# Atten4Vis/LW-DETR

Hardware: AMD Instinct MI355X
Metric: images/sec (higher is better)
Workload: dtype fp16; 1 GPU; LW-DETR-small inference forward + PostProcess, 640x640, batch 32/GPU, fp16, random-init weights (synthetic COCO-shaped input); global_batch=32, per_gpu_batch=32, parallelism=dp1, collective=none, launch_chains=2

## Files before the change

include/lwdetr_hip.h:

```cpp
#ifndef LWDETR_HIP_H
#define LWDETR_HIP_H
#include <stdint.h>
#ifdef __cplusplus
extern "C" {
#endif

#define LWDETR_OK 0
#define LWDETR_ERR_BAD_ARG (-1)
#define LWDETR_ERR_UNSUPPORTED (-2)
#define LWDETR_ERR_LAUNCH (-3)

int lwdetr_msda_forward(const void* value, const int64_t* shapes, const int64_t* level_start, const void* loc,
                        const void* attn, void* out, int B, int S, int M, int D, int L, int Q, int P, int dtype,
                        void* hip_stream);

int lwdetr_msda_backward(const void* value, const int64_t* shapes, const int64_t* level_start, const void* loc,
                         const void* attn, const void* grad_out, void* grad_value, void* grad_loc, void* grad_attn,
                         int B, int S, int M, int D, int L, int Q, int P, int dtype, void* hip_stream);

int lwdetr_msda_fused_forward(const void* value, const int64_t* shapes, const int64_t* level_start, const void* oa,
                              long ld_oa, int logit_col, const float* ref_boxes, const float* valid_ratios, void* out,
                              int B, int S, int M, int D, int L, int Q, int P, int dtype, void* hip_stream);

typedef struct {
    int winmajor;
    int Hp, Wp, Twp;
} lwdetr_tok_layout;

enum { LWDETR_A_PLAIN = 0, LWDETR_A_CONV3x3 = 1, LWDETR_A_PATCH16 = 2 };
enum { LWDETR_ACT_NONE = 0, LWDETR_ACT_RELU = 1, LWDETR_ACT_GELU = 2, LWDETR_ACT_SILU = 3 };
enum { LWDETR_OUT_LINEAR = 0, LWDETR_OUT_HEADS = 1, LWDETR_OUT_HEADS_T = 2, LWDETR_OUT_TOKMAP = 3,
       LWDETR_OUT_DECONV2x2 = 4 };

typedef struct {
    void* out;
    void* out2;
    const void* res;
    const float* bias;
    const float* gamma;
    const uint8_t* rowmask;
    float scale;
    int act;
    int mode;
    int n_begin, n_end;
    long ldo, ld2, ldres;
    int res_mod;
    int rowmask_after;
    int p0, p1, p2;
    lwdetr_tok_layout in_tok, out_tok;
    long out_batch_stride;
    long out_row_offset;
    const float* ln_stats;
    const float* ln_colsum;
} lwdetr_gemm_seg;

typedef struct {
    const void* A; const void* A2;
    const void* W;
    int M, N, K;
    long lda;
    int a_mode;
    lwdetr_tok_layout a_tok;
    int conv_cin, conv_stride, a_col0, conv_hout, conv_wout;
    int img_h, img_w;
    int nseg;
    lwdetr_gemm_seg seg[3];
    void* splitk_ws;
    int splitk;
} lwdetr_gemm_desc;

int lwdetr_gemm(const lwdetr_gemm_desc* desc, int dtype, void* hip_stream);
int lwdetr_gemm_few(const lwdetr_gemm_desc* desc, int dtype, void* hip_stream);
int lwdetr_row_stats(const void* x, long ldx, long M, int C, float eps, float* stats, int dtype, void* hip_stream);
void lwdetr_gemm_tuning(int big_mode);
int lwdetr_has_experiments(void);
void lwdetr_gemm_pt_tuning(int pt_mode);
long lwdetr_gemm_pt_count(void);
int lwdetr_gemm_path_counts(long* out, int n);
const char* lwdetr_gemm_path_name(int i);

typedef struct {
    const void* Q;
    const void* K;
    const void* VT;
    void* out;
    long ldo;
    int B, heads, hd, Tp;
    int seqs_per_img;
    int seq_tok_stride;
    int keys_per_seq;
    int sub_stride, sub_len;
    int kind;
    int vt_slack;
} lwdetr_attn_desc;

int lwdetr_attention(const lwdetr_attn_desc* desc, int dtype, void* hip_stream);
void lwdetr_attention_tuning(int lds_mode);
void lwdetr_attention_tuning_cfg(int cfg);

int lwdetr_layernorm(const void* x, long ldx, const float* gamma, const float* beta, void* out, long ldo, long M,
                     int C, float eps, long rows_per_batch, long out_batch_rows, long out_row_offset, int dtype,
                     void* hip_stream);

int lwdetr_layernorm_chain(const void* x, long ldx, const float* gamma1, const float* beta1, float eps1, void* out1, long ldo1,
                           const float* gamma2, const float* beta2, float eps2, void* out2, long ldo2, long M, int C,
                           int dtype, void* hip_stream);

int lwdetr_ffn_splits(long M, int C, int hid, int dtype);
int lwdetr_ffn_partial(const void* x, long ldx, const void* w1, const float* b1, const void* w2_chunked, float* partial, long M,
                       int C, int hid, int dtype, void* hip_stream);
int lwdetr_ffn_finish(const void* x, long ldx, const float* partial, int splits, const float* b2, const float* gamma1,
                      const float* beta1, float eps1, void* out1, long ldo1, const float* gamma2, const float* beta2, float eps2,
                      void* out2, long ldo2, long M, int C, int dtype, void* hip_stream);

int lwdetr_mlp_fused(void* x, long ldx, const void* w1_folded, const float* b1_folded, const void* w2_chunked,
                     const float* b2, const float* gamma2, void* out2, long ld2, float* stats_out, long M, int C,
                     float eps, float eps_next, const void* att, long ldatt, const void* wp, const float* bp,
                     const float* gamma1, const void* wqkv_next, const float* bqkv_next, void* q_out, void* k_out,
                     void* vt_out, float qscale, int heads, int hd, int Tp, int dtype, void* hip_stream);

int lwdetr_vit_block_few(void* x, long ldx, const void* w1_frag, const float* b1_folded, const void* w2_chunked, const float* b2,
                         const float* gamma2, void* out2, long ld2, float* stats_out, long M, int C, float eps, float eps_next,
                         const void* att, long ldatt, const void* wp_frag, const float* bp, const float* gamma1,
                         const void* wqkv_frag_next, const float* bqkv_next, void* q_out, void* k_out, void* vt_out, float qscale,
                         int heads, int hd, int Tp, int dtype, void* hip_stream);

int lwdetr_vit_path_counts(long* out, int n);
const char* lwdetr_vit_path_name(int i);

int lwdetr_msda_path_counts(long* out, int n);
const char* lwdetr_msda_path_name(int i);
long lwdetr_vit_block_stream_bytes(int C, int has_qkv);
long lwdetr_vit_block_vec_floats(int C);
int lwdetr_vit_block(void* x, long ldx, const void* att, long ldatt, const void* wstream, const float* vec, void* out2,
                     long ld2, float* stats_out, long M, int C, float eps, float eps_next, int has_qkv, void* q_out,
                     void* k_out, void* vt_out, float qscale, int heads, int hd, int Tp, int dtype, void* hip_stream);

long lwdetr_enc_chain_vec_floats(int D, int k5);
long lwdetr_enc_chain_pieces(int D, int k5, int nl);
long lwdetr_enc_chain_class_cols(int ncls);
long lwdetr_enc_chain_vec_floats_cls(int D, int k5, int ncls);
long lwdetr_enc_chain_pieces_cls(int D, int k5, int nl, int ncls);
int lwdetr_enc_chain_check(const void* in, long ld_in, int k5, void* memory, void* om, void* cls, long ld_cls, float* cls_max,
                           void* const* values, int nl, const unsigned char* rowvalid, const unsigned char* notpad,
                           const void* wstream, const float* vec, long M, int D, int npix, int S, int lsi, long total_rows,
                           int ncls, int dtype);
int lwdetr_enc_chain(const void* in, long ld_in, int k5, void* memory, void* om, void* cls, long ld_cls, float* cls_max,
                     void* const* values, int nl, const unsigned char* rowvalid, const unsigned char* notpad,
                     const void* wstream, const float* vec, long M, int D, int npix, int S, int lsi, long total_rows,
                     int ncls, float eps_p, float eps_e, int dtype, void* hip_stream);

enum { LWDETR_CHAIN_FULL = 0, LWDETR_CHAIN_SIDE = 1 };
enum { LWDETR_CHAIN_RES = 1, LWDETR_CHAIN_RELU = 2, LWDETR_CHAIN_LN = 4, LWDETR_CHAIN_STORE = 8, LWDETR_CHAIN_ADDQ = 16 };
typedef struct { int kind; int n; int flags; float eps; void* out; long ldo; } lwdetr_chain_stage;
typedef struct {
    const void* in; long ld_in; int k_in;
    const void* res; long ld_res;
    const void* qpos; long ld_q;
    const void* wstream; const float* vec;
    long M; int D; int nst;
    lwdetr_chain_stage st[6];
} lwdetr_chain_desc;
long lwdetr_row_chain_pieces(const lwdetr_chain_desc* desc);
long lwdetr_row_chain_vec_floats(const lwdetr_chain_desc* desc);
int lwdetr_row_chain(const lwdetr_chain_desc* desc, int dtype, void* hip_stream);

long lwdetr_vit_qkv_stream_bytes(int C);
long lwdetr_vit_qkv_vec_floats(int C);
int lwdetr_vit_qkv(const void* x, long ldx, const void* wstream, const float* vec, long M, int C, float eps, void* q_out,
                   void* k_out, void* vt_out, float qscale, int heads, int hd, int Tp, int dtype, void* hip_stream);

long lwdetr_vit_stem_stream_bytes(int C);
long lwdetr_vit_stem_vec_floats(int C);
int lwdetr_vit_stem(const void* img, int B, int img_h, int img_w, int Hp, int Wp, int Twp, const void* pos, long ldpos, void* x,
                    long ldx, const void* wstream, const float* vec, long M, int C, float eps, void* q_out, void* k_out,
                    void* vt_out, float qscale, int heads, int hd, int dtype, void* hip_stream);

int lwdetr_select_gather(const void* om, const void* enc_cls, long ldc, const float* props, const int64_t* idx,
                         void* om_sel, void* logits_out, float* props_sel, int B, int S, int d, int nq, int ncls,
                         int dtype, void* hip_stream);
int lwdetr_decoder_inputs(const void* enc_delta, const float* props_sel, const float* refpoint, const float* valid_ratios,
                          int L, const void* query_feat, const float* dim_t, void* enc_boxes_out, float* ref_out,
                          void* sine_out, void* xdec_out, int B, int nq, int d, int dtype, void* hip_stream);
int lwdetr_box_reparam(const void* delta, const float* ref, long ref_rows, void* out, long R, int dtype, void* hip_stream);
int lwdetr_finalize_outputs(const void* delta, const float* ref, long ref_rows, void* coord_out, long R, const void* logits_pad,
                            long ldc, int ncls, void* logits_out, long out_layer_rows, int dtype, void* hip_stream);

int lwdetr_rowmax(const void* x, long ld, long rows, int ncols, float* out, int dtype, void* hip_stream);
int lwdetr_topk(const void* x, int B, int N, int K, int64_t* idx_out, float* val_out, int dtype, void* hip_stream);
int lwdetr_postprocess(const void* logits, const void* boxes, const float* target_sizes, int B, int nq, int ncls, int K,
                       float* scores, int64_t* labels, float* out_boxes, int dtype, void* hip_stream);
int lwdetr_postprocess_packed(const void* logits, const void* boxes, const float* target_sizes, int B, int nq, int ncls, int K,
                              float* packed, int dtype, void* hip_stream);

typedef struct {
    const uint8_t* src;
    int height, width;
    long row_stride;
    int xbounds_off, xcoef_off, xksize;
    int ybounds_off, ycoef_off, yksize;
    long tmp_off;
} lwdetr_resize_image;
int lwdetr_resize_normalize(const lwdetr_resize_image* images, int B, int max_height, const int32_t* tables, uint8_t* tmp,
                            const float* lut, void* out, int S, int dtype, void* hip_stream);

int lwdetr_tuning_set(const char* name, long value, int is_set);

int lwdetr_prof_enable(int on);
int lwdetr_prof_num_kernels(void);
const char* lwdetr_prof_kernel_name(int kid);
int lwdetr_prof_collect(double* ms, double* flops, double* bytes, long long* count, int n);

#ifdef __cplusplus
}
#endif
#endif
```

lw-detr_amd/csrc/attention.hip:

```cpp
#include "common.h"
#include <cstdlib>

namespace {

__device__ __forceinline__ float xor16_max(float v) {
    const auto r = __builtin_amdgcn_permlane16_swap(__float_as_uint(v), __float_as_uint(v), false, false);
    return fmaxf(__uint_as_float(r[0]), __uint_as_float(r[1]));
}
__device__ __forceinline__ float xor32_max(float v) {
    const auto r = __builtin_amdgcn_permlane32_swap(__float_as_uint(v), __float_as_uint(v), false, false);
    return fmaxf(__uint_as_float(r[0]), __uint_as_float(r[1]));
}
__device__ __forceinline__ float xor16_sum(float v) {
    const auto r = __builtin_amdgcn_permlane16_swap(__float_as_uint(v), __float_as_uint(v), false, false);
    return __uint_as_float(r[0]) + __uint_as_float(r[1]);
}
__device__ __forceinline__ float xor32_sum(float v) {
    const auto r = __builtin_amdgcn_permlane32_swap(__float_as_uint(v), __float_as_uint(v), false, false);
    return __uint_as_float(r[0]) + __uint_as_float(r[1]);
}

__device__ __forceinline__ float max3(float a, float b, float c) { return __builtin_fmaxf(__builtin_fmaxf(a, b), c); }

#ifndef LWDETR_ATTN_ABL
#define LWDETR_ATTN_ABL 0
#endif

template <typename T, int HD, int QT, bool SHORT = false>
__global__ __launch_bounds__(256) void attn_kernel(const lwdetr_attn_desc p) {
    typedef typename Vec<T>::v8 V8;
    typedef typename Vec<T>::v4 V4;
    constexpr int NC = HD >= 32 ? HD / 32 : 1;
    constexpr int DT = HD / 16;
    const int lane = threadIdx.x & 63, wave = threadIdx.x >> 6;
    const int l15 = lane & 15, g = lane >> 4;
    const int head = blockIdx.y, seq = blockIdx.z;
    const int q0 = (blockIdx.x * 4 + wave) * 16 * QT;
    if (q0 >= p.keys_per_seq) return;
    const int b = seq / p.seqs_per_img, w = seq - b * p.seqs_per_img;
    const long tok0 = (long)w * p.seq_tok_stride;
    const long bh = (long)b * p.heads + head;
    const T* __restrict__ Qb = (const T*)p.Q + (bh * p.Tp + tok0) * HD;
    const T* __restrict__ Kb = (const T*)p.K + (bh * p.Tp + tok0) * HD;
    const T* __restrict__ Vb = (const T*)p.VT + bh * HD * (long)p.Tp + tok0;
    const int nkeys = p.keys_per_seq;
    const int last = nkeys - 1;

    V8 q8[QT][NC]; V4 q4[QT];
#pragma unroll
    for (int t = 0; t < QT; ++t) {
        int q = q0 + t * 16 + l15; q = q < last ? q : last;
        if (HD >= 32) {
#pragma unroll
            for (int c = 0; c < NC; ++c) q8[t][c] = *(const V8*)(Qb + (long)q * HD + c * 32 + g * 8);
        } else {
            q4[t] = *(const V4*)(Qb + (long)q * HD + g * 4);
        }
    }

    f32x4 o[QT][DT], lsum[QT];
    f32x4 negm[QT];
#pragma unroll
    for (int t = 0; t < QT; ++t) {
        negm[t] = f32x4{0.f, 0.f, 0.f, 0.f}; lsum[t] = f32x4{0.f, 0.f, 0.f, 0.f};
#pragma unroll
        for (int dt = 0; dt < DT; ++dt) o[t][dt] = f32x4{0.f, 0.f, 0.f, 0.f};
    }
    V8 ones;
#pragma unroll
    for (int e = 0; e < 8; ++e) ones[e] = from_f32<T>(1.f);

    const bool holes = p.sub_len < p.sub_stride;
    constexpr float RESCALE_THR = 8.f;

    struct KV { V8 k8[2][NC]; V4 k4[2]; V8 v[DT]; };
    auto load_k = [&](int k0, KV& f) {
#pragma unroll
        for (int kt = 0; kt < 2; ++kt) {
            int key = k0 + 8 * (l15 >> 2) + 4 * kt + (l15 & 3); key = key < last ? key : last;
            if (HD >= 32) {
#pragma unroll
                for (int c = 0; c < NC; ++c) f.k8[kt][c] = *(const V8*)(Kb + (long)key * HD + c * 32 + g * 8);
            } else {
                f.k4[kt] = *(const V4*)(Kb + (long)key * HD + g * 4);
            }
        }
    };
    auto load_v = [&](int k0, KV& f) {
        int kv = k0 + g * 8;
        kv = kv + 7 < nkeys ? kv : (nkeys - 8);
        const bool shift4 = k0 + g * 8 - kv == 4;
#pragma unroll
        for (int dt = 0; dt < DT; ++dt) {
            V8 v = *(const V8*)(Vb + (long)(dt * 16 + l15) * p.Tp + kv);
            if (shift4) {
#pragma unroll
                for (int e = 0; e < 4; ++e) v[e] = v[4 + e];
            }
            f.v[dt] = v;
        }
    };
    auto load_kv = [&](int k0, KV& f) { load_k(k0, f); load_v(k0, f); };

    auto qk_tile = [&](const KV& f, int t, f32x4 (&st)[2]) {
#pragma unroll
        for (int kt = 0; kt < 2; ++kt) {
            f32x4 a = negm[t];
            if (LWDETR_ATTN_ABL & 4) { a[0] += to_f32<T>(f.k4[kt][0]); st[kt] = a; continue; }
            if (HD >= 32) {
#pragma unroll
                for (int c = 0; c < NC; ++c) a = Mma<T>::k32(f.k8[kt][c], q8[t][c], a);
            } else {
                a = Mma<T>::k16(f.k4[kt], q4[t], a);
            }
            st[kt] = a;
        }
    };
    auto softmax_head = [&](f32x4 (&s)[QT][2], int k0) {
        if (k0 + 32 > nkeys || holes) {
#pragma unroll
            for (int kt = 0; kt < 2; ++kt)
#pragma unroll
                for (int r = 0; r < 4; ++r) {
                    const int key = k0 + g * 8 + kt * 4 + r;
                    const int sub = holes ? key % p.sub_stride : 0;
                    const bool ok = (key < nkeys) & (sub < p.sub_len);
#pragma unroll
                    for (int t = 0; t < QT; ++t) s[t][kt][r] = ok ? s[t][kt][r] : -INFINITY;
                }
        }
        float lmax[QT];
#pragma unroll
        for (int t = 0; t < QT; ++t) {
            lmax[t] = max3(s[t][0][0], s[t][0][1], s[t][0][2]);
            lmax[t] = max3(lmax[t], s[t][0][3], s[t][1][0]);
            lmax[t] = max3(lmax[t], s[t][1][1], s[t][1][2]);
            lmax[t] = max3(lmax[t], s[t][1][3], s[t][1][3]);
        }
        if (LWDETR_ATTN_ABL & 2) { for (int t = 0; t < QT; ++t) lmax[t] = s[t][0][0]; }
        float lall = lmax[0];
#pragma unroll
        for (int t = 1; t + 1 < QT; t += 2) lall = max3(lall, lmax[t], lmax[t + 1]);
        if (QT % 2 == 0) lall = max3(lall, lmax[QT - 1], lmax[QT - 1]);
        const bool need = k0 == 0 || lall > RESCALE_THR;
        if (__any(need)) {
#pragma unroll
            for (int t = 0; t < QT; ++t) {
                float mx = xor32_max(xor16_max(lmax[t]));
                mx = k0 == 0 ? mx : fmaxf(mx, 0.f);
                const float alpha = __builtin_amdgcn_exp2f(-mx);
                negm[t] -= mx;
#pragma unroll
                for (int kt = 0; kt < 2; ++kt) s[t][kt] -= mx;
                lsum[t] *= alpha;
#pragma unroll
                for (int dt = 0; dt < DT; ++dt) o[t][dt] *= alpha;
            }
        }
    };
    auto pv_tile = [&](const KV& f, int t, const f32x4 (&st)[2]) {
        V8 pf;
#pragma unroll
        for (int kt = 0; kt < 2; ++kt)
#pragma unroll
            for (int r = 0; r < 4; ++r) {
                const float e = (LWDETR_ATTN_ABL & 1) ? st[kt][r] : __builtin_amdgcn_exp2f(st[kt][r]);
                pf[kt * 4 + r] = from_f32<T>(e);
            }
        if (LWDETR_ATTN_ABL & 8) { lsum[t][0] += to_f32<T>(pf[0]) + to_f32<T>(pf[5]); return; }
        lsum[t] = Mma<T>::k32(ones, pf, lsum[t]);
#pragma unroll
        for (int dt = 0; dt < DT; ++dt) o[t][dt] = Mma<T>::k32(f.v[dt], pf, o[t][dt]);
    };
    auto step = [&](const KV& f, int k0) {
        f32x4 s[QT][2];
#pragma unroll
        for (int t = 0; t < QT; ++t) qk_tile(f, t, s[t]);
        softmax_head(s, k0);
#pragma unroll
        for (int t = 0; t < QT; ++t) pv_tile(f, t, s[t]);
    };

    if constexpr (SHORT) {
        KV f4[4];
#pragma unroll
        for (int i = 0; i < 4; ++i) load_kv(32 * i, f4[i]);
#pragma unroll
        for (int i = 0; i < 4; ++i) {
            if (32 * i >= nkeys) break;
            step(f4[i], 32 * i);
        }
    } else {
    KV fa, fb;
    if (nkeys >= 512) {
        load_kv(0, fa);
        for (int k0 = 0;;) {
            load_kv(k0 + 32, fb);
            step(fa, k0);
            k0 += 32;
            if (k0 >= nkeys) break;
            load_kv(k0 + 32, fa);
            step(fb, k0);
            k0 += 32;
            if (k0 >= nkeys) break;
        }
    } else {
        load_kv(0, fa);
        for (int k0 = 0;;) {
            if (k0 + 32 < nkeys) load_kv(k0 + 32, fb);
            step(fa, k0);
            k0 += 32;
            if (k0 >= nkeys) break;
            if (k0 + 32 < nkeys) load_kv(k0 + 32, fa);
            step(fb, k0);
            k0 += 32;
            if (k0 >= nkeys) break;
        }
    }
    }

    T* __restrict__ out = (T*)p.out;
#pragma unroll
    for (int t = 0; t < QT; ++t) {
        const float l = lsum[t][0];
        const float inv = 1.f / l;
        const int q = q0 + t * 16 + l15;
        if (q < nkeys) {
            T* orow = out + ((long)b * p.Tp + tok0 + q) * p.ldo + head * HD;
#pragma unroll
            for (int dt = 0; dt < DT; ++dt) {
                V4 ov;
#pragma unroll
                for (int r = 0; r < 4; ++r) ov[r] = from_f32<T>(o[t][dt][r] * inv);
                *(V4*)(orow + dt * 16 + g * 4) = ov;
            }
        }
    }
}


template <typename T> struct Mma32;
template <> struct Mma32<f16> {
    static __device__ __forceinline__ f32x16 k16(f16x8 a, f16x8 b, f32x16 c) {
        return __builtin_amdgcn_mfma_f32_32x32x16_f16(a, b, c, 0, 0, 0);
    }
    static __device__ __forceinline__ float dot2(f16x8 p, int i, float c) {
        typedef _Float16 h2 __attribute__((ext_vector_type(2)));
        const h2 a = {p[2 * i], p[2 * i + 1]}, one = {(f16)1.f, (f16)1.f};
        return __builtin_amdgcn_fdot2(a, one, c, false);
    }
};
template <> struct Mma32<bf16> {
    static __device__ __forceinline__ f32x16 k16(bf16x8 a, bf16x8 b, f32x16 c) {
        return __builtin_amdgcn_mfma_f32_32x32x16_bf16(a, b, c, 0, 0, 0);
    }
    static __device__ __forceinline__ float dot2(bf16x8 p, int i, float c) {
        typedef __bf16 b2 __attribute__((ext_vector_type(2)));
        const b2 a = {p[2 * i], p[2 * i + 1]}, one = {(bf16)1.f, (bf16)1.f};
        return __builtin_amdgcn_fdot2_f32_bf16(a, one, c, false);
    }
};

__device__ __attribute__((aligned(16))) unsigned int g_attn_zero16[4];

__device__ __forceinline__ void attn_dma16(const void* src, unsigned lds_base) {
    asm volatile("s_mov_b32 m0, %0\n\ts_nop 0\n\tglobal_load_lds_dwordx4 %1, off" :: "s"(lds_base), "v"(src) : "memory");
}
template <int N> __device__ __forceinline__ void attn_wait_vmcnt() { asm volatile("s_waitcnt vmcnt(%0)" ::"n"(N) : "memory"); }

template <typename T, int HD, int QT, int NW, int U>
__global__ __launch_bounds__(NW * 64) void attn_lds_kernel(const lwdetr_attn_desc p) {
    typedef typename Vec<T>::v8 V8;
    constexpr int NC = HD / 16;
    constexpr int RT = HD > 32 ? HD / 32 : 1;
    constexpr int RB = HD * 2;
    constexpr int CPR = RB / 16, RPB = 256 / RB;
    constexpr int KB = 64;
    constexpr int KIMG = KB * RB, VIMG = RT * 32 * 128, STAGE = KIMG + VIMG;
    constexpr int NKP = KIMG / 1024, NVP = HD * 128 / 1024, NP = NKP + NVP;
    constexpr int SSTAGE = U * STAGE;
    constexpr int PPW = (U * NP + NW - 1) / NW;
    constexpr int NST = 3;
    constexpr int QW = 32 * QT, QWG = QW * NW;
    constexpr float RESCALE_THR = 8.f;
    __shared__ __attribute__((aligned(16))) char smem[NST * SSTAGE + 1024];

    const int lane = threadIdx.x & 63;
    const int wave = __builtin_amdgcn_readfirstlane(threadIdx.x >> 6);
    const int m = lane & 31, h = lane >> 5;
    const int nkeys = p.keys_per_seq;
    const int wgs_per_seq = (nkeys + QWG - 1) / QWG;
    int wid;
    {
        const int nwg = gridDim.x, bid = blockIdx.x, q = nwg >> 3, r = nwg & 7, xcd = bid & 7;
        wid = (xcd < r ? xcd * (q + 1) : r * (q + 1) + (xcd - r) * q) + (bid >> 3);
    }
    const int qblk = wid % wgs_per_seq;
    const int rest = wid / wgs_per_seq;
    const int head = rest % p.heads, seq = rest / p.heads;
    const int b = seq / p.seqs_per_img, w = seq - b * p.seqs_per_img;
    const long tok0 = (long)w * p.seq_tok_stride;
    const long bh = (long)b * p.heads + head;
    const T* __restrict__ Qb = (const T*)p.Q + (bh * p.Tp + tok0) * HD;
    const T* __restrict__ Kb = (const T*)p.K + (bh * p.Tp + tok0) * HD;
    const T* __restrict__ Vb = (const T*)p.VT + bh * HD * (long)p.Tp + tok0;
    const int q0 = qblk * QWG + wave * QW;
    const bool active = q0 < nkeys;
    const int nblk = (nkeys + KB - 1) / KB;
    const int nstep = (nblk + U - 1) / U;

    V8 qf[QT][NC];
#pragma unroll
    for (int t = 0; t < QT; ++t) {
        int q = q0 + t * 32 + m; q = q < nkeys ? q : nkeys - 1;
#pragma unroll
        for (int c = 0; c < NC; ++c) qf[t][c] = *(const V8*)(Qb + (long)q * HD + c * 16 + h * 8);
    }

    const T* src0[PPW]; const T* srct[PPW]; int sstep[PPW]; unsigned dst0[PPW]; bool real[PPW]; int sub[PPW];
    const unsigned lds0 = (unsigned)(uintptr_t)(__attribute__((address_space(3))) const void*)smem;
    const unsigned dummy_dst = lds0 + NST * SSTAGE;
    const int kt0 = (nblk - 1) * KB;
#pragma unroll
    for (int j = 0; j < PPW; ++j) {
        const int ii = wave + j * NW;
        const int i = ii % NP;
        sub[j] = ii / NP;
        if (ii >= U * NP) {
            src0[j] = (const T*)g_attn_zero16; srct[j] = src0[j]; sstep[j] = 0; dst0[j] = 0; real[j] = false;
        } else if (i < NKP) {
            const int off = i * 1024 + lane * 16;
            const int key = off / RB, slot = (off % RB) / 16;
            const int chunk = slot ^ ((key / RPB) & (CPR - 1));
            src0[j] = Kb + key * HD + chunk * 8; sstep[j] = KB * HD; dst0[j] = sub[j] * STAGE + i * 1024; real[j] = true;
            const int kc = kt0 + key < nkeys ? kt0 + key : nkeys - 1;
            srct[j] = Kb + (long)kc * HD + chunk * 8;
        } else {
            const int v = i - NKP;
            const int row = 8 * v + (lane >> 3), slot = lane & 7;
            const int chunk = slot ^ ((row >> 1) & 7);
            src0[j] = Vb + (long)row * p.Tp + chunk * 8; sstep[j] = KB; dst0[j] = sub[j] * STAGE + KIMG + v * 1024; real[j] = true;
            srct[j] = kt0 + chunk * 8 < nkeys ? src0[j] + kt0 : (const T*)g_attn_zero16;
        }
    }
    auto issue = [&](int step, int slot_) {
        const unsigned sb = lds0 + slot_ * SSTAGE;
#pragma unroll
        for (int j = 0; j < PPW; ++j) {
            const int blk = step * U + sub[j];
            const bool live = real[j] && blk < nblk;
            const T* src = !live ? (const T*)g_attn_zero16 : (blk == nblk - 1 ? srct[j] : src0[j] + (long)blk * sstep[j]);
            attn_dma16(src, __builtin_amdgcn_readfirstlane(live ? sb + dst0[j] : dummy_dst));
        }
    };

    if (HD == 16) {
        V8 one8, zero8;
#pragma unroll
        for (int e = 0; e < 8; ++e) { one8[e] = from_f32<T>(1.f); zero8[e] = from_f32<T>(0.f); }
        for (int i = threadIdx.x; i < NST * U * 16 * 8; i += NW * 64) {
            const int st = i / 128, r = (i % 128) / 8, sl = i % 8;
            *(V8*)(smem + st * STAGE + KIMG + (16 + r) * 128 + sl * 16) = r == 0 ? one8 : zero8;
        }
    }

    const int km = (m & ~12) | ((m & 4) << 1) | ((m & 8) >> 1);
    int kofs[NC];
#pragma unroll
    for (int c = 0; c < NC; ++c) kofs[c] = km * RB + (((2 * c + h) ^ ((km / RPB) & (CPR - 1))) << 4);
    int vofs[2][2];
#pragma unroll
    for (int t = 0; t < 2; ++t)
#pragma unroll
        for (int s = 0; s < 2; ++s) vofs[t][s] = KIMG + m * 128 + (((4 * t + 2 * s + h) ^ ((m >> 1) & 7)) << 4);

    f32x16 o[QT][RT], negm[QT];
    float lsum[QT];
#pragma unroll
    for (int t = 0; t < QT; ++t) {
        lsum[t] = 0.f;
#pragma unroll
        for (int e = 0; e < 16; ++e) negm[t][e] = 0.f;
#pragma unroll
        for (int r = 0; r < RT; ++r)
#pragma unroll
            for (int e = 0; e < 16; ++e) o[t][r][e] = 0.f;
    }
    const bool holes = p.sub_len < p.sub_stride;
    int res0 = 0;

// ... 384 lines not shown
    const int kid = p.kind == 0 ? KID_ATTN_WINDOW : (p.kind == 1 ? KID_ATTN_GLOBAL : KID_ATTN_DECODER);
    ProfScope ps(kid, flops, bytes, st);
    hipLaunchKernelGGL((attn_win_kernel<T, HD>), dim3((unsigned)((npairs + 3) / 4)), dim3(256), 0, st, p);
    return lwdetr_check_launch();
}

#ifdef LWDETR_EXPERIMENTS
template <typename T>
__global__ __launch_bounds__(256) void attn_wtile_kernel(const lwdetr_attn_desc p) {
    constexpr int HD = 16;
    typedef typename Vec<T>::v8 V8;
    typedef typename Vec<T>::v4 V4;
    typedef unsigned u32x4v __attribute__((ext_vector_type(4)));
    typedef unsigned u32x2 __attribute__((ext_vector_type(2)));
    static_assert(sizeof(T) == 2, "16-bit types");
    extern __shared__ __attribute__((aligned(16))) char wt_smem[];
    const int tid = threadIdx.x, lane = tid & 63, wave = tid >> 6, l31 = lane & 31, h = lane >> 5;
    const int w = (int)(blockIdx.x % (unsigned)p.seqs_per_img), b = (int)(blockIdx.x / (unsigned)p.seqs_per_img);
    const long tok0 = (long)w * p.seq_tok_stride;
    const int nkeys = p.keys_per_seq, last = nkeys - 1;
    const int nvalid = p.sub_len < nkeys ? p.sub_len : nkeys;
    const int nqt = (nkeys + 31) >> 5, nkt = (nvalid + 31) >> 5, nch = (nvalid + 15) >> 4;
    const int C = p.heads * HD;
    const int VLD = ((nkeys + 7) & ~7) + 8;
    const int OLD = C + 8;
    T* vs = (T*)wt_smem;
    T* os = vs + (size_t)C * VLD;

    auto load_qk = [&](int head, V8 (&kf)[4], V8 (&qf)[4]) {
        const long bh = (long)b * p.heads + head;
        const T* __restrict__ Qb = (const T*)p.Q + (bh * p.Tp + tok0) * HD;
        const T* __restrict__ Kb = (const T*)p.K + (bh * p.Tp + tok0) * HD;
#pragma unroll
        for (int t = 0; t < 4; ++t) {
            int r = t * 32 + l31; r = r < last ? r : last;
            kf[t] = *(const V8*)(Kb + (long)r * HD + h * 8);
            qf[t] = *(const V8*)(Qb + (long)r * HD + h * 8);
        }
    };
    V8 kf[4], qf[4];
    int head = wave;
    if (head < p.heads) load_qk(head, kf, qf);
    {
        const int ppr = nkeys >> 2, total = C * ppr;
        const T* __restrict__ Vw = (const T*)p.VT + (long)b * C * (long)p.Tp + tok0;
        for (int i = tid; i < total; i += 256) {
            const int row = i / ppr, pc = i - row * ppr;
            *(V4*)(vs + (size_t)row * VLD + 4 * pc) = *(const V4*)(Vw + (long)row * p.Tp + 4 * pc);
        }
    }
    __syncthreads();

    while (head < p.heads) {
        const int nh = head + 4;
        V8 kn[4], qn[4];
        if (nh < p.heads) load_qk(nh, kn, qn);
        const T* vrow = vs + (size_t)(head * HD + (l31 & 15)) * VLD;
#pragma unroll
        for (int qt = 0; qt < 4; ++qt) {
            if (qt >= nqt) break;
            f32x16 sc[4];
#pragma unroll
            for (int kt = 0; kt < 4; ++kt) {
                if (kt >= nkt) break;
                f32x16 a;
#pragma unroll
                for (int e = 0; e < 16; ++e) a[e] = 0.f;
                a = Mma32<T>::k16(kf[kt], qf[qt], a);
                if (kt * 32 + 32 > nvalid) {
                    asm volatile("; ragged key tile");
#pragma unroll
                    for (int e = 0; e < 16; ++e) a[e] = kt * 32 + 8 * (e >> 2) + 4 * h + (e & 3) < nvalid ? a[e] : -INFINITY;
                }
                sc[kt] = a;
            }
            float mx = -INFINITY;
#pragma unroll
            for (int kt = 0; kt < 4; ++kt) {
                if (kt >= nkt) break;
                float lm = max3(sc[kt][0], sc[kt][1], sc[kt][2]);
#pragma unroll
                for (int e = 3; e < 15; e += 2) lm = max3(lm, sc[kt][e], sc[kt][e + 1]);
                mx = max3(mx, lm, sc[kt][15]);
            }
            mx = xor32_max(mx);
            f32x16 o;
#pragma unroll
            for (int e = 0; e < 16; ++e) o[e] = 0.f;
#pragma unroll
            for (int c = 0; c < 8; ++c) {
                if (c >= nch) break;
                V8 pf, vf;
#pragma unroll
                for (int e = 0; e < 8; ++e) pf[e] = from_f32<T>(__builtin_amdgcn_exp2f(sc[c >> 1][8 * (c & 1) + e] - mx));
                if (l31 >= 16) {
#pragma unroll
                    for (int e = 0; e < 8; ++e) vf[e] = from_f32<T>(l31 == 16 ? 1.f : 0.f);
                } else {
                    int k0 = 16 * c + 4 * h, k1 = k0 + 8;
                    k0 = k0 + 4 <= nkeys ? k0 : nkeys - 4; k1 = k1 + 4 <= nkeys ? k1 : nkeys - 4;
                    const V4 lo = *(const V4*)(vrow + k0), hi = *(const V4*)(vrow + k1);
#pragma unroll
                    for (int e = 0; e < 4; ++e) { vf[e] = lo[e]; vf[4 + e] = hi[e]; }
                }
                o = Mma32<T>::k16(vf, pf, o);
            }
            const auto rr = __builtin_amdgcn_permlane32_swap(__float_as_uint(o[8]), __float_as_uint(o[8]), false, false);
            const float inv = 1.f / (h == 0 ? o[8] : __uint_as_float(rr[0]));
            V4 lo, hi;
#pragma unroll
            for (int e = 0; e < 4; ++e) { lo[e] = from_f32<T>(o[e] * inv); hi[e] = from_f32<T>(o[4 + e] * inv); }
            const u32x2 lu = __builtin_bit_cast(u32x2, lo), hu = __builtin_bit_cast(u32x2, hi);
            const auto s0 = __builtin_amdgcn_permlane32_swap(lu[0], hu[0], false, false);
            const auto s1 = __builtin_amdgcn_permlane32_swap(lu[1], hu[1], false, false);
            const u32x4v st = {s0[0], s1[0], s0[1], s1[1]};
            const int q = qt * 32 + l31;
            if (q < nkeys) *(u32x4v*)(os + (size_t)q * OLD + head * HD + 8 * h) = st;
        }
#pragma unroll
        for (int t = 0; t < 4; ++t) { kf[t] = kn[t]; qf[t] = qn[t]; }
        head = nh;
    }
    __syncthreads();
    {
        const int cpr = C >> 3, total = nkeys * cpr;
        T* __restrict__ out = (T*)p.out + ((long)b * p.Tp + tok0) * p.ldo;
        for (int i = tid; i < total; i += 256) {
            const int row = i / cpr, c8 = i - row * cpr;
            *(u32x4v*)(out + (long)row * p.ldo + 8 * c8) = *(const u32x4v*)(os + (size_t)row * OLD + 8 * c8);
        }
    }
}

template <typename T>
int launch_wtile(const lwdetr_attn_desc& p, hipStream_t st) {
    const int C = p.heads * 16, VLD = ((p.keys_per_seq + 7) & ~7) + 8;
    const size_t lds = ((size_t)C * VLD + (size_t)p.keys_per_seq * (C + 8)) * sizeof(T);
    static signed char state[16] = {};
    int dev = 0;
    if (hipGetDevice(&dev) != hipSuccess || dev < 0 || dev >= 16) return LWDETR_ERR_UNSUPPORTED;
    if (state[dev] == 0)
        state[dev] = hipFuncSetAttribute((const void*)attn_wtile_kernel<T>, hipFuncAttributeMaxDynamicSharedMemorySize, 128 * 1024) == hipSuccess ? 1 : -1;
    if (state[dev] < 0) { (void)hipGetLastError(); return LWDETR_ERR_UNSUPPORTED; }
    const double nseq = (double)p.B * p.seqs_per_img;
    const double flops = 4.0 * nseq * p.heads * (double)p.keys_per_seq * p.keys_per_seq * 16;
    const double bytes = 4.0 * nseq * p.heads * p.keys_per_seq * 16 * sizeof(T);
    const int kid = p.kind == 0 ? KID_ATTN_WINDOW : (p.kind == 1 ? KID_ATTN_GLOBAL : KID_ATTN_DECODER);
    ProfScope ps(kid, flops, bytes, st);
    hipLaunchKernelGGL((attn_wtile_kernel<T>), dim3((unsigned)(p.B * p.seqs_per_img)), dim3(256), lds, st, p);
    return lwdetr_check_launch();
}
#endif

template <typename T, int HD, int QT>
int launch_qt(const lwdetr_attn_desc& p, hipStream_t st) {
    const int units = (p.keys_per_seq + 16 * QT - 1) / (16 * QT);
    dim3 grid((units + 3) / 4, p.heads, p.B * p.seqs_per_img);
    const double nseq = (double)p.B * p.seqs_per_img;
    const double flops = 4.0 * nseq * p.heads * (double)p.keys_per_seq * p.keys_per_seq * HD;
    const double bytes = 4.0 * nseq * p.heads * p.keys_per_seq * HD * sizeof(T);
    const int kid = p.kind == 0 ? KID_ATTN_WINDOW : (p.kind == 1 ? KID_ATTN_GLOBAL : KID_ATTN_DECODER);
    ProfScope ps(kid, flops, bytes, st);
    const bool short_off = lwdetr_knob(KNOB_ATTN_SHORT, 1) == 0;
    if constexpr (QT == 2 && sizeof(T) == 2) {
        if (p.keys_per_seq <= 128 && !short_off) {
            hipLaunchKernelGGL((attn_kernel<T, HD, QT, true>), grid, dim3(256), 0, st, p);
            return lwdetr_check_launch();
        }
    }
    hipLaunchKernelGGL((attn_kernel<T, HD, QT>), grid, dim3(256), 0, st, p);
    return lwdetr_check_launch();
}

template <typename T, int HD>
int launch(const lwdetr_attn_desc& p, hipStream_t st) {
    if constexpr (sizeof(T) == 2 && HD == 16) {
#ifdef LWDETR_EXPERIMENTS
        const int wmode = (int)lwdetr_knob(KNOB_ATTN_WTILE, 0);
        const int C = p.heads * 16, VLD = ((p.keys_per_seq + 7) & ~7) + 8;
        const size_t lds = ((size_t)C * VLD + (size_t)p.keys_per_seq * (C + 8)) * sizeof(T);
        if (wmode != 0 && p.keys_per_seq <= 128 && p.keys_per_seq >= 4 && p.keys_per_seq % 4 == 0 && p.Tp % 4 == 0 &&
            p.sub_stride >= p.keys_per_seq && p.ldo % 8 == 0 && ((size_t)p.out & 15) == 0 &&
            ((size_t)p.VT & 7) == 0 && p.seq_tok_stride % 4 == 0 && lds <= 128 * 1024) {
            const int rc = launch_wtile<T>(p, st);
            if (rc != LWDETR_ERR_UNSUPPORTED) return rc;
        }
#endif
    }
    if constexpr (sizeof(T) == 2 && (HD == 16 || HD == 32)) {
        const int mode = (int)lwdetr_knob(KNOB_ATTN_WIN, 2);
        if (mode != 0 && (mode == 1 || HD == 32) && p.keys_per_seq <= 128 && p.sub_stride >= p.keys_per_seq && p.ldo % 8 == 0 &&
            ((size_t)p.out & 15) == 0 && (long)p.B * p.heads * p.seqs_per_img / 4 < 0x7fffffffL)
            return launch_win<T, HD>(p, st);
    }
    if (LdsPath<T, HD>::ok(p) && lds_path_applies(p)) return LdsPath<T, HD>::go(p, st);
    const long wgs4 = (long)((p.keys_per_seq + 255) / 256) * p.heads * p.B * p.seqs_per_img;
    const bool qt4 = lwdetr_knob_is_set(KNOB_ATTN_QT) ? lwdetr_knob(KNOB_ATTN_QT, 0) == 4 : (p.keys_per_seq >= 1024 && HD <= 32 && sizeof(T) == 2 && wgs4 >= 256);
    if (qt4) return launch_qt<T, HD, (HD <= 32 ? 4 : 2)>(p, st);
    return launch_qt<T, HD, 2>(p, st);
}

template <typename T>
int dispatch_hd(const lwdetr_attn_desc& p, hipStream_t st) {
    switch (p.hd) {
        case 16: return launch<T, 16>(p, st);
        case 32: return launch<T, 32>(p, st);
        case 64: return launch<T, 64>(p, st);
        default: return LWDETR_ERR_UNSUPPORTED;
    }
}

}

#ifdef LWDETR_ATTN_HD16_TU
extern "C" __attribute__((visibility("hidden"))) int lwdetr_attn_lds_hd16_impl(const lwdetr_attn_desc* p, int dtype, void* hip_stream, int cfg) {
    g_attn_lds_cfg = cfg;
    return dtype == DT_F16 ? launch_lds_cfg<f16, 16>(*p, (hipStream_t)hip_stream) : launch_lds_cfg<bf16, 16>(*p, (hipStream_t)hip_stream);
}
#else
extern "C" void lwdetr_attention_tuning(int lds_mode) { g_attn_lds_mode = lds_mode; }
extern "C" void lwdetr_attention_tuning_cfg(int cfg) { g_attn_lds_cfg = cfg; }

extern "C" int lwdetr_attention(const lwdetr_attn_desc* desc, int dtype, void* hip_stream) {
    if (!desc) return LWDETR_ERR_BAD_ARG;
    const lwdetr_attn_desc& p = *desc;
    if (!p.Q || !p.K || !p.VT || !p.out || p.B <= 0 || p.heads <= 0 || p.Tp <= 0 || p.Tp % 4 != 0) return LWDETR_ERR_BAD_ARG;
    if (p.seqs_per_img <= 0 || p.keys_per_seq < 8 || p.keys_per_seq % 4 != 0 || p.sub_stride <= 0 || p.sub_len <= 0 || p.sub_len > p.sub_stride)
        return LWDETR_ERR_BAD_ARG;
    if ((long)(p.seqs_per_img - 1) * p.seq_tok_stride + p.keys_per_seq > p.Tp) return LWDETR_ERR_BAD_ARG;
    if (p.seq_tok_stride % 4 != 0 || p.ldo % 4 != 0) return LWDETR_ERR_BAD_ARG;
    if ((long)p.B * p.seqs_per_img > 65535 || p.heads > 65535) return LWDETR_ERR_BAD_ARG;
    hipStream_t st = (hipStream_t)hip_stream;
    switch (dtype) {
        case DT_F32: return dispatch_hd<float>(p, st);
        case DT_F16: return dispatch_hd<f16>(p, st);
        case DT_BF16: return dispatch_hd<bf16>(p, st);
        default: return LWDETR_ERR_UNSUPPORTED;
    }
}
#endif
```

Baseline: 14400 images/sec.

## Add specialized head-dim-16 short-window attention kernel with lazy rescale

Adds a dedicated kernel for 16-bit, head-dim-16 attention with at most 128 keys, used by default in place of the generic short-sequence kernel. One block covers a whole sequence and head, with its 16-query tiles split across four waves. Each wave preloads all K/V fragments and runs K=16 MFMAs. The running max is rescaled only when it grows past a threshold, and row sums are accumulated with dot2 instructions instead of an MFMA against ones. It also allows 4-key sequences and adds an optional cycle-stamp instrumentation path, at the cost of more code paths and a separate translation unit for the launch.

```diff
diff --git a/include/lwdetr_hip.h b/include/lwdetr_hip.h
--- a/include/lwdetr_hip.h
+++ b/include/lwdetr_hip.h
@@ -97,6 +97,8 @@
 int lwdetr_attention(const lwdetr_attn_desc* desc, int dtype, void* hip_stream);
 void lwdetr_attention_tuning(int lds_mode);
 void lwdetr_attention_tuning_cfg(int cfg);
+void lwdetr_attention_win16(int mode);
+long lwdetr_attn_win16_count(void);
 
 int lwdetr_layernorm(const void* x, long ldx, const float* gamma, const float* beta, void* out, long ldo, long M,
                      int C, float eps, long rows_per_batch, long out_batch_rows, long out_row_offset, int dtype,
diff --git a/lw-detr_amd/csrc/attention.hip b/lw-detr_amd/csrc/attention.hip
--- a/lw-detr_amd/csrc/attention.hip
+++ b/lw-detr_amd/csrc/attention.hip
@@ -45,6 +45,10 @@
     const T* __restrict__ Vb = (const T*)p.VT + bh * HD * (long)p.Tp + tok0;
     const int nkeys = p.keys_per_seq;
     const int last = nkeys - 1;
+#ifdef LWDETR_ATTN_STAMP
+    unsigned long long stamp[4] = {__builtin_readcyclecounter(), 0, 0, 0};
+    const unsigned long long stamp_rt = __builtin_amdgcn_s_memrealtime();
+#endif
 
     V8 q8[QT][NC]; V4 q4[QT];
 #pragma unroll
@@ -185,11 +189,19 @@
         KV f4[4];
 #pragma unroll
         for (int i = 0; i < 4; ++i) load_kv(32 * i, f4[i]);
+#ifdef LWDETR_ATTN_STAMP
+        asm volatile("s_waitcnt vmcnt(0)" ::: "memory");
+        stamp[1] = __builtin_readcyclecounter();
+#endif
 #pragma unroll
         for (int i = 0; i < 4; ++i) {
             if (32 * i >= nkeys) break;
             step(f4[i], 32 * i);
         }
+#ifdef LWDETR_ATTN_STAMP
+        asm volatile("" :: "v"(o[0][0][0]), "v"(o[QT - 1][0][0]), "v"(lsum[0][0]) : "memory");
+        stamp[2] = __builtin_readcyclecounter();
+#endif
     } else {
     KV fa, fb;
     if (nkeys >= 512) {
@@ -236,6 +248,16 @@
             }
         }
     }
+#ifdef LWDETR_ATTN_STAMP
+    asm volatile("s_waitcnt vmcnt(0)" ::: "memory");
+    stamp[3] = __builtin_readcyclecounter();
+    if (lane == 0) {
+        typedef unsigned u4 __attribute__((ext_vector_type(4)));
+        const u4 sv = {(unsigned)(stamp[1] - stamp[0]), (unsigned)(stamp[2] - stamp[1]), (unsigned)(stamp[3] - stamp[2]),
+                       (unsigned)(__builtin_amdgcn_s_memrealtime() - stamp_rt)};
+        *(u4*)(out + ((long)b * p.Tp + tok0 + q0) * p.ldo + head * HD) = sv;
+    }
+#endif
 }
 
 
@@ -926,8 +948,264 @@
 }
 #endif
 
+template <typename T> struct W16KV {
+    typename Vec<T>::v4 k4[2];
+    typename Vec<T>::v8 v;
+};
+template <typename T> struct Dot2;
+template <> struct Dot2<f16> {
+    static __device__ __forceinline__ float go(f16 a, f16 b, float c) {
+        typedef _Float16 h2 __attribute__((ext_vector_type(2)));
+        return __builtin_amdgcn_fdot2(h2{a, b}, h2{(f16)1.f, (f16)1.f}, c, false);
+    }
+};
+template <> struct Dot2<bf16> {
+    static __device__ __forceinline__ float go(bf16 a, bf16 b, float c) {
+        typedef __bf16 b2 __attribute__((ext_vector_type(2)));
+        return __builtin_amdgcn_fdot2_f32_bf16(b2{a, b}, b2{(bf16)1.f, (bf16)1.f}, c, false);
+    }
+};
+
+template <typename T>
+__device__ __forceinline__ typename Vec<T>::v4 w16_load_q(const T* __restrict__ Qb, int q0, int nkeys, bool on, int lane) {
+    typedef typename Vec<T>::v4 V4;
+    V4 r;
+#pragma unroll
+    for (int e = 0; e < 4; ++e) r[e] = from_f32<T>(0.f);
+    const int q = q0 + (lane & 15);
+    if (on && q < nkeys) r = *(const V4*)(Qb + (unsigned)(q * 16 + (lane >> 4) * 4));
+    return r;
+}
+template <typename T>
+__device__ __forceinline__ W16KV<T> w16_load_kv(const lwdetr_attn_desc& p, const T* __restrict__ Kb, const T* __restrict__ Vb, int i, int lane) {
+    typedef typename Vec<T>::v8 V8;
+    typedef typename Vec<T>::v4 V4;
+    const int l15 = lane & 15, g = lane >> 4;
+    const int nkeys = p.keys_per_seq;
+    const int k0 = 32 * i, rem = nkeys - k0;
+    V4 zero4;
+#pragma unroll
+    for (int e = 0; e < 4; ++e) zero4[e] = from_f32<T>(0.f);
+    W16KV<T> f;
+    f.k4[0] = zero4; f.k4[1] = zero4;
+#pragma unroll
+    for (int e = 0; e < 8; ++e) f.v[e] = from_f32<T>(0.f);
+    if (rem >= 32) {
+#pragma unroll
+        for (int kt = 0; kt < 2; ++kt) f.k4[kt] = *(const V4*)(Kb + (unsigned)((k0 + 8 * (l15 >> 2) + 4 * kt + (l15 & 3)) * 16 + g * 4));
+        f.v = *(const V8*)(Vb + (unsigned)(l15 * p.Tp + k0 + g * 8));
+    } else if (rem > 16) {
+#pragma unroll
+        for (int kt = 0; kt < 2; ++kt) {
+            const int key = k0 + 8 * (l15 >> 2) + 4 * kt + (l15 & 3);
+            if (key < nkeys) f.k4[kt] = *(const V4*)(Kb + (unsigned)(key * 16 + g * 4));
+        }
+        const int kv = k0 + g * 8;
+        V4 lo = zero4, hi = zero4;
+        if (kv < nkeys) lo = *(const V4*)(Vb + (unsigned)(l15 * p.Tp + kv));
+        if (kv + 4 < nkeys) hi = *(const V4*)(Vb + (unsigned)(l15 * p.Tp + kv + 4));
+#pragma unroll
+        for (int e = 0; e < 4; ++e) { f.v[e] = lo[e]; f.v[4 + e] = hi[e]; }
+    } else if (rem > 0) {
+        if (k0 + l15 < nkeys) f.k4[0] = *(const V4*)(Kb + (unsigned)((k0 + l15) * 16 + g * 4));
+        if (k0 + g * 4 < nkeys) {
+            const V4 lo = *(const V4*)(Vb + (unsigned)(l15 * p.Tp + k0 + g * 4));
+#pragma unroll
+            for (int e = 0; e < 4; ++e) f.v[e] = lo[e];
+        }
+    }
+    return f;
+}
+
+template <typename T, int QT, typename KVF>
+__device__ __forceinline__ void w16_run(const typename Vec<T>::v4 (&q4)[QT], KVF&& kv, const lwdetr_attn_desc& p, T* __restrict__ ob, int q0, int lane) {
+    typedef typename Vec<T>::v8 V8;
+    typedef typename Vec<T>::v4 V4;
+    const int l15 = lane & 15, g = lane >> 4;
+    const int nkeys = p.keys_per_seq;
+    const bool holes = p.sub_len < p.sub_stride;
+    constexpr float RESCALE_THR = 8.f;
+    f32x4 o[QT], negm[QT];
+    float dsum[QT];
+#pragma unroll
+    for (int t = 0; t < QT; ++t) { negm[t] = f32x4{0.f, 0.f, 0.f, 0.f}; o[t] = negm[t]; dsum[t] = 0.f; }
+
+    auto rescale = [&](const float (&lmax)[QT], bool first, auto&& shift) {
+        float lall = lmax[0];
+#pragma unroll
+        for (int t = 1; t < QT; ++t) lall = __builtin_fmaxf(lall, lmax[t]);
+        if (__any(first || lall > RESCALE_THR)) {
+#pragma unroll
+            for (int t = 0; t < QT; ++t) {
+                float mx = xor32_max(xor16_max(lmax[t]));
+                mx = first ? mx : fmaxf(mx, 0.f);
+                const float alpha = __builtin_amdgcn_exp2f(-mx);
+                negm[t] -= mx;
+                shift(t, mx);
+                dsum[t] *= alpha;
+                o[t] *= alpha;
+            }
+        }
+    };
+    auto step32 = [&](const W16KV<T>& f, int k0) {
+        f32x4 s[QT][2];
+#pragma unroll
+        for (int t = 0; t < QT; ++t)
+#pragma unroll
+            for (int kt = 0; kt < 2; ++kt) s[t][kt] = Mma<T>::k16(f.k4[kt], q4[t], negm[t]);
+        if (k0 + 32 > nkeys || holes) {
+#pragma unroll
+            for (int kt = 0; kt < 2; ++kt)
+#pragma unroll
+                for (int r = 0; r < 4; ++r) {
+                    const int key = k0 + g * 8 + kt * 4 + r;
+                    const int sub = holes ? key % p.sub_stride : 0;
+                    const bool ok = (key < nkeys) & (sub < p.sub_len);
+#pragma unroll
+                    for (int t = 0; t < QT; ++t) s[t][kt][r] = ok ? s[t][kt][r] : -INFINITY;
+                }
+        }
+        float lmax[QT];
+#pragma unroll
+        for (int t = 0; t < QT; ++t) {
+            lmax[t] = max3(s[t][0][0], s[t][0][1], s[t][0][2]);
+            lmax[t] = max3(lmax[t], s[t][0][3], s[t][1][0]);
+            lmax[t] = max3(lmax[t], s[t][1][1], s[t][1][2]);
+            lmax[t] = __builtin_fmaxf(lmax[t], s[t][1][3]);
+        }
+        rescale(lmax, k0 == 0, [&](int t, float mx) { s[t][0] -= mx; s[t][1] -= mx; });
+#pragma unroll
+        for (int t = 0; t < QT; ++t) {
+            V8 pf;
+#pragma unroll
+            for (int kt = 0; kt < 2; ++kt)
+#pragma unroll
+                for (int r = 0; r < 4; ++r) pf[kt * 4 + r] = from_f32<T>(__builtin_amdgcn_exp2f(s[t][kt][r]));
+#pragma unroll
+            for (int e = 0; e < 8; e += 2) dsum[t] = Dot2<T>::go(pf[e], pf[e + 1], dsum[t]);
+            o[t] = Mma<T>::k32(f.v, pf, o[t]);
+        }
+    };
+    auto step16 = [&](const W16KV<T>& f, int k0) {
+        f32x4 s[QT];
+#pragma unroll
+        for (int t = 0; t < QT; ++t) s[t] = Mma<T>::k16(f.k4[0], q4[t], negm[t]);
+        if (k0 + 16 > nkeys || holes) {
+#pragma unroll
+            for (int r = 0; r < 4; ++r) {
+                const int key = k0 + g * 4 + r;
+                const int sub = holes ? key % p.sub_stride : 0;
+                const bool ok = (key < nkeys) & (sub < p.sub_len);
+#pragma unroll
+                for (int t = 0; t < QT; ++t) s[t][r] = ok ? s[t][r] : -INFINITY;
+            }
+        }
+        float lmax[QT];
+#pragma unroll
+        for (int t = 0; t < QT; ++t) lmax[t] = __builtin_fmaxf(max3(s[t][0], s[t][1], s[t][2]), s[t][3]);
+        rescale(lmax, k0 == 0, [&](int t, float mx) { s[t] -= mx; });
+        V4 vlo;
+#pragma unroll
+        for (int e = 0; e < 4; ++e) vlo[e] = f.v[e];
+#pragma unroll
+        for (int t = 0; t < QT; ++t) {
+            V4 pf;
+#pragma unroll
+            for (int r = 0; r < 4; ++r) pf[r] = from_f32<T>(__builtin_amdgcn_exp2f(s[t][r]));
+            dsum[t] = Dot2<T>::go(pf[0], pf[1], dsum[t]);
+            dsum[t] = Dot2<T>::go(pf[2], pf[3], dsum[t]);
+            o[t] = Mma<T>::k16(vlo, pf, o[t]);
+        }
+    };
+#pragma unroll
+    for (int i = 0; i < 4; ++i) {
+        const int rem = nkeys - 32 * i;
+        if (rem <= 0) break;
+        const W16KV<T> f = kv(i);
+        if (rem > 16) step32(f, 32 * i); else step16(f, 32 * i);
+    }
+#pragma unroll
+    for (int t = 0; t < QT; ++t) {
+        const float inv = 1.f / xor32_sum(xor16_sum(dsum[t]));
+        const int q = q0 + t * 16 + l15;
+        if (q < nkeys) {
+            V4 ov;
+#pragma unroll
+            for (int r = 0; r < 4; ++r) ov[r] = from_f32<T>(o[t][r] * inv);
+            *(V4*)(ob + (long)q * p.ldo + g * 4) = ov;
+        }
+    }
+}
+
+template <typename T, int QT>
+__device__ __forceinline__ void w16_item(const lwdetr_attn_desc& p, int b, long tok0, int head, int q0, int lane) {
+    const long bh = (long)b * p.heads + head;
+    const T* __restrict__ Qb = (const T*)p.Q + (bh * p.Tp + tok0) * 16;
+    const T* __restrict__ Kb = (const T*)p.K + (bh * p.Tp + tok0) * 16;
+    const T* __restrict__ Vb = (const T*)p.VT + bh * 16 * (long)p.Tp + tok0;
+    typename Vec<T>::v4 q4[QT];
+    W16KV<T> f[4];
+#pragma unroll
+    for (int t = 0; t < QT; ++t) q4[t] = w16_load_q<T>(Qb, q0 + 16 * t, p.keys_per_seq, true, lane);
+#pragma unroll
+    for (int i = 0; i < 4; ++i) f[i] = w16_load_kv<T>(p, Kb, Vb, i, lane);
+    w16_run<T, QT>(q4, [&](int i) { return f[i]; }, p, (T*)p.out + ((long)b * p.Tp + tok0) * p.ldo + head * 16, q0, lane);
+}
+
+template <typename T>
+__global__ __launch_bounds__(256) __attribute__((amdgpu_waves_per_eu(std::is_same<T, f16>::value ? 6 : 1))) void attn_w16_kernel(const lwdetr_attn_desc p) {
+    static_assert(sizeof(T) == 2, "16-bit types");
+    const int lane = threadIdx.x & 63;
+    const int wave = __builtin_amdgcn_readfirstlane(threadIdx.x >> 6);
+    const int head0 = blockIdx.y, seq = blockIdx.z;
+    const int ntile = (p.keys_per_seq + 15) >> 4;
+    const int base = ntile >> 2, extra = ntile & 3;
+    const int cnt = base + (wave < extra ? 1 : 0);
+    const int q0 = 16 * (wave * base + (wave < extra ? wave : extra));
+    const int b = seq / p.seqs_per_img, w = seq - b * p.seqs_per_img;
+    const long tok0 = (long)w * p.seq_tok_stride;
+    switch (cnt) {
+        case 1: w16_item<T, 1>(p, b, tok0, head0, q0, lane); break;
+        case 2: w16_item<T, 2>(p, b, tok0, head0, q0, lane); break;
+        default: break;
+    }
+}
+
+#ifndef LWDETR_ATTN_HD16_TU
+int g_attn_win16_mode = -1;
+long g_attn_win16_launches = 0;
+static int attn_win16_mode() {
+    static const int env = [] { const char* e = getenv("LWDETR_ATTN_WIN16"); return e && *e ? atoi(e) : 1; }();
+    return g_attn_win16_mode >= 0 ? g_attn_win16_mode : env;
+}
+#else
+template <typename T>
+int launch_w16(const lwdetr_attn_desc& p, hipStream_t st) {
+    const double nseq = (double)p.B * p.seqs_per_img;
+    const double flops = 4.0 * nseq * p.heads * (double)p.keys_per_seq * p.keys_per_seq * 16;
+    const double bytes = 4.0 * nseq * p.heads * p.keys_per_seq * 16 * sizeof(T);
+    const int kid = p.kind == 0 ? KID_ATTN_WINDOW : (p.kind == 1 ? KID_ATTN_GLOBAL : KID_ATTN_DECODER);
+    ProfScope ps(kid, flops, bytes, st);
+    hipLaunchKernelGGL((attn_w16_kernel<T>), dim3(1, p.heads, p.B * p.seqs_per_img), dim3(256), 0, st, p);
+    return lwdetr_check_launch();
+}
+#endif
+}
+extern "C" __attribute__((visibility("hidden"))) int lwdetr_attn_w16_impl(const lwdetr_attn_desc* p, int dtype, void* hip_stream);
+namespace {
+
 template <typename T, int HD, int QT>
 int launch_qt(const lwdetr_attn_desc& p, hipStream_t st) {
+    const bool short_off = lwdetr_knob(KNOB_ATTN_SHORT, 1) == 0;
+#ifndef LWDETR_ATTN_HD16_TU
+    if constexpr (QT == 2 && sizeof(T) == 2 && HD == 16) {
+        if (p.keys_per_seq <= 128 && !short_off && attn_win16_mode() != 0) {
+            const int rc = lwdetr_attn_w16_impl(&p, std::is_same<T, f16>::value ? DT_F16 : DT_BF16, (void*)st);
+            if (rc == LWDETR_OK) ++g_attn_win16_launches;
+            return rc;
+        }
+    }
+#endif
     const int units = (p.keys_per_seq + 16 * QT - 1) / (16 * QT);
     dim3 grid((units + 3) / 4, p.heads, p.B * p.seqs_per_img);
     const double nseq = (double)p.B * p.seqs_per_img;
@@ -935,7 +1213,6 @@
     const double bytes = 4.0 * nseq * p.heads * p.keys_per_seq * HD * sizeof(T);
     const int kid = p.kind == 0 ? KID_ATTN_WINDOW : (p.kind == 1 ? KID_ATTN_GLOBAL : KID_ATTN_DECODER);
     ProfScope ps(kid, flops, bytes, st);
-    const bool short_off = lwdetr_knob(KNOB_ATTN_SHORT, 1) == 0;
     if constexpr (QT == 2 && sizeof(T) == 2) {
         if (p.keys_per_seq <= 128 && !short_off) {
             hipLaunchKernelGGL((attn_kernel<T, HD, QT, true>), grid, dim3(256), 0, st, p);
@@ -991,20 +1268,27 @@
     g_attn_lds_cfg = cfg;
     return dtype == DT_F16 ? launch_lds_cfg<f16, 16>(*p, (hipStream_t)hip_stream) : launch_lds_cfg<bf16, 16>(*p, (hipStream_t)hip_stream);
 }
+extern "C" __attribute__((visibility("hidden"))) int lwdetr_attn_w16_impl(const lwdetr_attn_desc* p, int dtype, void* hip_stream) {
+    return dtype == DT_F16 ? launch_w16<f16>(*p, (hipStream_t)hip_stream) : launch_w16<bf16>(*p, (hipStream_t)hip_stream);
+}
 #else
 extern "C" void lwdetr_attention_tuning(int lds_mode) { g_attn_lds_mode = lds_mode; }
+extern "C" void lwdetr_attention_win16(int mode) { g_attn_win16_mode = mode; }
+extern "C" long lwdetr_attn_win16_count(void) { return g_attn_win16_launches; }
 extern "C" void lwdetr_attention_tuning_cfg(int cfg) { g_attn_lds_cfg = cfg; }
 
 extern "C" int lwdetr_attention(const lwdetr_attn_desc* desc, int dtype, void* hip_stream) {
     if (!desc) return LWDETR_ERR_BAD_ARG;
     const lwdetr_attn_desc& p = *desc;
     if (!p.Q || !p.K || !p.VT || !p.out || p.B <= 0 || p.heads <= 0 || p.Tp <= 0 || p.Tp % 4 != 0) return LWDETR_ERR_BAD_ARG;
-    if (p.seqs_per_img <= 0 || p.keys_per_seq < 8 || p.keys_per_seq % 4 != 0 || p.sub_stride <= 0 || p.sub_len <= 0 || p.sub_len > p.sub_stride)
+    const bool four = p.keys_per_seq == 4 && p.hd == 16 && (dtype == DT_F16 || dtype == DT_BF16) && attn_win16_mode() != 0 && lwdetr_knob(KNOB_ATTN_SHORT, 1) != 0;
+    if (p.seqs_per_img <= 0 || (p.keys_per_seq < 8 && !four) || p.keys_per_seq % 4 != 0 || p.sub_stride <= 0 || p.sub_len <= 0 || p.sub_len > p.sub_stride)
         return LWDETR_ERR_BAD_ARG;
     if ((long)(p.seqs_per_img - 1) * p.seq_tok_stride + p.keys_per_seq > p.Tp) return LWDETR_ERR_BAD_ARG;
     if (p.seq_tok_stride % 4 != 0 || p.ldo % 4 != 0) return LWDETR_ERR_BAD_ARG;
     if ((long)p.B * p.seqs_per_img > 65535 || p.heads > 65535) return LWDETR_ERR_BAD_ARG;
     hipStream_t st = (hipStream_t)hip_stream;
+    if (four) return dtype == DT_F16 ? launch_qt<f16, 16, 2>(p, st) : launch_qt<bf16, 16, 2>(p, st);
     switch (dtype) {
         case DT_F32: return dispatch_hd<float>(p, st);
         case DT_F16: return dispatch_hd<f16>(p, st);
```

Measured after the change: 14490 images/sec, median of 6. No clear change (+0.6%).
